# SimonZeng7108/efficientsam3

Hardware: NVIDIA H100
Metric: encoder images/sec @1024^2 (EV-M student forward) (higher is better)
Workload: dtype bf16

## Files before the change

efficientsam3_b200/csrc/gemm_tc.cu:

```cuda
#include <cstdio>
#include <cstdlib>

#include "ptx.cuh"

namespace es3 {

struct GemmArgs {
  int M, N;
  int num_kb;
  int kb_per_tap;
  int tiles_n;
  int conv;
  int H, W, TW, TH, tiles_w, tiles_h;
  int Ctap;
  const float* scale;
  const float* bias;
  int act;
  const bf16* residual;
  long long ldr;
  void* out;
  long long ldo;
  int out_f32;
  int res_f32;
  const float2* rope;
  int rope_cols, rope_H, rope_W, rope_win;
  int ct_cout, ct_H, ct_W;
  int act_after_res;
  int dbg;
};

constexpr int BM = 128;
constexpr int BK = 64;

constexpr int EPI_WARPS = 4;
constexpr int EPI_WARP0 = 4;
constexpr int TMA_WARP = EPI_WARP0 + EPI_WARPS;
constexpr int GEMM_THREADS = (TMA_WARP + 1) * 32;
template <int BN, int STAGES, int CPR>
struct GemmSmem {
  static constexpr int A_BYTES = BM * BK * 2;
  static constexpr int B_BYTES = BN * BK * 2;
  static constexpr int STAGE_BYTES = A_BYTES + B_BYTES;
  static constexpr int ACC_LD = BN + 8;
  static constexpr int OFF_ACC = STAGES * STAGE_BYTES;
  static constexpr int OFF_EPI = OFF_ACC + BM * ACC_LD * 4;
  static constexpr int EPI_TILE_BYTES = 32 * 16 * CPR;
  static constexpr int TOTAL = OFF_EPI + EPI_WARPS * EPI_TILE_BYTES;
};

template <int CPR>
__device__ __forceinline__ uint8_t* epi_chunk(uint8_t* tile, int r, int c) {
  if constexpr (CPR == 4) return tile + r * 64 + ((c ^ ((r >> 1) & 3)) << 4);
  else return tile + r * 32 + ((c ^ ((r >> 2) & 1)) << 4);
}

template <int CPR>
__device__ __forceinline__ void epi_store_rows(uint8_t* tile, const uint4* mine, uint8_t* gbase, long long my_off_bytes,
                                               bool my_valid, int lane) {
  constexpr int RPI = 32 / CPR;
#pragma unroll
  for (int p = 0; p < 4 / CPR; ++p) {
#pragma unroll
    for (int j = 0; j < CPR; ++j) *reinterpret_cast<uint4*>(epi_chunk<CPR>(tile, lane, j)) = mine[p * CPR + j];
    __syncwarp();
#pragma unroll
    for (int j = 0; j < CPR; ++j) {
      const int r = j * RPI + lane / CPR, c = lane % CPR;
      const long long off = __shfl_sync(0xffffffffu, my_off_bytes, r);
      const int ok = __shfl_sync(0xffffffffu, (int)my_valid, r);
      const uint4 u = *reinterpret_cast<const uint4*>(epi_chunk<CPR>(tile, r, c));
      if (ok) *reinterpret_cast<uint4*>(gbase + off + (p * CPR + c) * 16) = u;
    }
    __syncwarp();
  }
}

template <int CPR>
__device__ __forceinline__ void epi_load_rows(uint8_t* tile, uint4* mine, const uint8_t* gbase, long long my_off_bytes,
                                              bool my_valid, int lane) {
  constexpr int RPI = 32 / CPR;
#pragma unroll
  for (int p = 0; p < 4 / CPR; ++p) {
#pragma unroll
    for (int j = 0; j < CPR; ++j) {
      const int r = j * RPI + lane / CPR, c = lane % CPR;
      const long long off = __shfl_sync(0xffffffffu, my_off_bytes, r);
      const int ok = __shfl_sync(0xffffffffu, (int)my_valid, r);
      uint4 u = make_uint4(0u, 0u, 0u, 0u);
      if (ok) u = __ldg(reinterpret_cast<const uint4*>(gbase + off + (p * CPR + c) * 16));
      *reinterpret_cast<uint4*>(epi_chunk<CPR>(tile, r, c)) = u;
    }
    __syncwarp();
#pragma unroll
    for (int j = 0; j < CPR; ++j) mine[p * CPR + j] = *reinterpret_cast<const uint4*>(epi_chunk<CPR>(tile, lane, j));
    __syncwarp();
  }
}

template <int BN, int STAGES, int ACT, int CPR>
__global__ void __launch_bounds__(GEMM_THREADS, 1) gemm_tc_kernel(const __grid_constant__ CUtensorMap tmA,
                                                               const __grid_constant__ CUtensorMap tmB,
                                                               const GemmArgs args, const int num_tiles) {
  static_assert(BN == 32 || BN == 64 || BN == 128, "one warpgroup holds 128 x BN fp32 accumulators in registers");
  extern __shared__ __align__(1024) uint8_t smem[];
  __shared__ __align__(8) uint64_t full_bar[STAGES];
  __shared__ __align__(8) uint64_t empty_bar[STAGES];
  __shared__ __align__(8) uint64_t acc_full_bar;
  __shared__ __align__(8) uint64_t acc_empty_bar;

  using L = GemmSmem<BN, STAGES, CPR>;
  float* acc_s = reinterpret_cast<float*>(smem + L::OFF_ACC);

  const int warp = threadIdx.x >> 5;
  const int lane = threadIdx.x & 31;

  if (threadIdx.x == 0) {
    if (ptx::smem_u32(smem) & 1023u) { printf("es3: gemm_tc dynamic smem base not 1024-byte aligned\n"); __trap(); }
    ptx::prefetch_tmap(&tmA);
    ptx::prefetch_tmap(&tmB);
#pragma unroll
    for (int s = 0; s < STAGES; ++s) {
      ptx::mbar_init(&full_bar[s], 1);
      ptx::mbar_init(&empty_bar[s], 4);
    }
    ptx::mbar_init(&acc_full_bar, 4);
    ptx::mbar_init(&acc_empty_bar, EPI_WARPS);
    ptx::fence_mbar_init();
  }
  __syncthreads();
  const int per_img = args.tiles_w * args.tiles_h;

  if (warp == TMA_WARP) {
    if (lane == 0) {
      int stage = 0;
      uint32_t phase = 0;
      for (int tile = blockIdx.x; tile < num_tiles; tile += gridDim.x) {
        const int n0 = (args.dbg & 8) ? 0 : (tile % args.tiles_n) * BN;
        const int m_tile = (args.dbg & 8) ? 0 : tile / args.tiles_n;
        int img = 0, h0 = 0, w0 = 0;
        if (args.conv) {
          img = m_tile / per_img;
          const int t = m_tile % per_img;
          h0 = (t / args.tiles_w) * args.TH;
          w0 = (t % args.tiles_w) * args.TW;
        }
        for (int kb = 0; kb < args.num_kb; ++kb) {
          ptx::mbar_wait(&empty_bar[stage], phase ^ 1);
          uint8_t* sa = smem + stage * L::STAGE_BYTES;
          uint8_t* sb = sa + L::A_BYTES;
          ptx::mbar_arrive_expect_tx(&full_bar[stage], L::STAGE_BYTES);
          if (args.conv) {
            const int tap = kb / args.kb_per_tap;
            const int kc = kb - tap * args.kb_per_tap;
            const int dy = tap / 3 - 1, dx = tap % 3 - 1;
            ptx::tma_load_4d(&tmA, &full_bar[stage], sa, kc * BK, w0 + dx, h0 + dy, img);
            ptx::tma_load_2d(&tmB, &full_bar[stage], sb, tap * args.Ctap + kc * BK, n0);
          } else {
            ptx::tma_load_2d(&tmA, &full_bar[stage], sa, kb * BK, m_tile * BM);
            ptx::tma_load_2d(&tmB, &full_bar[stage], sb, kb * BK, n0);
          }
          if (++stage == STAGES) { stage = 0; phase ^= 1; }
        }
      }
    }
  } else if (warp < EPI_WARP0) {
    float d[2][BN / 2];
    int stage = 0;
    uint32_t phase = 0;
    uint32_t acc_phase = 0;
    for (int tile = blockIdx.x; tile < num_tiles; tile += gridDim.x) {
      int prev = -1;
      for (int kb = 0; kb < args.num_kb; ++kb) {
        ptx::mbar_wait(&full_bar[stage], phase);
        const uint32_t sa = ptx::smem_u32(smem + stage * L::STAGE_BYTES);
        const uint32_t sb = sa + L::A_BYTES;
        ptx::wg_fence();
#pragma unroll
        for (int k = 0; k < BK / 16; ++k) {
          const uint64_t db = ptx::make_desc_sw128(sb + k * 32);
#pragma unroll
          for (int h = 0; h < 2; ++h) {
            const uint64_t da = ptx::make_desc_sw128(sa + h * 8192 + k * 32);
            if constexpr (BN == 128) ptx::wgmma_m64n128<0, 0>(d[h], da, db, (kb | k) != 0);
            else if constexpr (BN == 64) ptx::wgmma_m64n64<0, 0>(d[h], da, db, (kb | k) != 0);
            else ptx::wgmma_m64n32<0, 0>(d[h], da, db, (kb | k) != 0);
          }
        }
        ptx::wg_commit();
        ptx::wg_wait<1>();
        if (prev >= 0 && lane == 0) ptx::mbar_arrive(&empty_bar[prev]);
        prev = stage;
        if (++stage == STAGES) { stage = 0; phase ^= 1; }
      }
      ptx::wg_wait<0>();
      ptx::wg_fence_regs<BN>(&d[0][0]);
      if (prev >= 0 && lane == 0) ptx::mbar_arrive(&empty_bar[prev]);
      ptx::mbar_wait(&acc_empty_bar, acc_phase ^ 1);
#pragma unroll
      for (int h = 0; h < 2; ++h)
#pragma unroll
        for (int i = 0; i < BN / 2; i += 2) {
          const int row = h * 64 + ptx::wg_frag_row(warp, lane, i), col = ptx::wg_frag_col(lane, i);
          *reinterpret_cast<float2*>(acc_s + row * L::ACC_LD + col) = make_float2(d[h][i], d[h][i + 1]);
        }
      __syncwarp();
      if (lane == 0) ptx::mbar_arrive(&acc_full_bar);
      acc_phase ^= 1;
    }
  } else {
    const int q = warp - EPI_WARP0;
    const int r = q * 32 + lane;
    uint8_t* epi_tile = smem + L::OFF_EPI + q * L::EPI_TILE_BYTES;
    uint32_t acc_phase = 0;
    for (int tile = blockIdx.x; tile < num_tiles; tile += gridDim.x) {
      const int n0 = (tile % args.tiles_n) * BN;
      const int m_tile = tile / args.tiles_n;
      bool valid;
      long long row_off;
      const bool dbg_nostore = (args.dbg & 1) != 0;
      if (args.conv) {
        const int img = m_tile / per_img;
        const int t = m_tile % per_img;
        const int h0 = (t / args.tiles_w) * args.TH, w0 = (t % args.tiles_w) * args.TW;
        const int dy = r / args.TW, dx = r - dy * args.TW;
        const int h = h0 + dy, w = w0 + dx;
        valid = (h < args.H) && (w < args.W);
        row_off = ((long long)img * args.H + h) * args.W + w;
      } else {
        const long long m = (long long)m_tile * BM + r;
        valid = m < args.M;
        row_off = m;
      }

      if (dbg_nostore) valid = false;
      ptx::mbar_wait(&acc_full_bar, acc_phase);

#pragma unroll 1
      for (int c = 0; c < BN / 32; ++c) {
        if (args.dbg & 4) break;
        uint32_t v[32];
        if (args.dbg & 2) {
#pragma unroll
          for (int j = 0; j < 32; ++j) v[j] = __float_as_uint((float)(r + j));
        } else {
          const uint4* src = reinterpret_cast<const uint4*>(acc_s + r * L::ACC_LD + c * 32);
#pragma unroll
          for (int j = 0; j < 8; ++j) {
            const uint4 u = src[j];
            v[4 * j] = u.x; v[4 * j + 1] = u.y; v[4 * j + 2] = u.z; v[4 * j + 3] = u.w;
          }
        }
        const int nb = n0 + c * 32;
        if (valid && nb < args.N && nb + 32 > args.N) {
          const int ncols = args.N - nb;
          const long long out_off = row_off * args.ldo + nb, res_off = row_off * args.ldr + nb;
#pragma unroll
          for (int j = 0; j < 32; ++j) {
            if (j < ncols) {
              float x = __uint_as_float(v[j]);
              if (args.scale != nullptr) x *= __ldg(args.scale + nb + j);
              if (args.bias != nullptr) x += __ldg(args.bias + nb + j);
              if (!args.act_after_res) x = es3_act_t<ACT>(x);
              if (args.residual != nullptr)
                x += args.res_f32 ? __ldg(reinterpret_cast<const float*>(args.residual) + res_off + j)
                                  : __bfloat162float(args.residual[res_off + j]);
              if (args.act_after_res) x = es3_act_t<ACT>(x);
              if (args.out_f32) reinterpret_cast<float*>(args.out)[out_off + j] = x;
              else reinterpret_cast<bf16*>(args.out)[out_off + j] = __float2bfloat16(x);
            }
          }
        } else if (nb + 32 <= args.N) {
          float f[32];
          if (args.scale != nullptr) {
            const float4* sc4 = reinterpret_cast<const float4*>(args.scale + nb);
#pragma unroll
            for (int j = 0; j < 8; ++j) {
              const float4 sc = __ldg(sc4 + j);
              f[4 * j + 0] = __uint_as_float(v[4 * j + 0]) * sc.x;
              f[4 * j + 1] = __uint_as_float(v[4 * j + 1]) * sc.y;
              f[4 * j + 2] = __uint_as_float(v[4 * j + 2]) * sc.z;
              f[4 * j + 3] = __uint_as_float(v[4 * j + 3]) * sc.w;
            }
          } else {
#pragma unroll
            for (int j = 0; j < 32; ++j) f[j] = __uint_as_float(v[j]);
          }
          if (args.bias != nullptr) {
            const float4* bi4 = reinterpret_cast<const float4*>(args.bias + nb);
#pragma unroll
            for (int j = 0; j < 8; ++j) {
              const float4 bi = __ldg(bi4 + j);
              f[4 * j + 0] += bi.x; f[4 * j + 1] += bi.y; f[4 * j + 2] += bi.z; f[4 * j + 3] += bi.w;
            }
          }
          long long out_off = row_off * args.ldo + nb, res_off = row_off * args.ldr + nb;
          if (args.ct_cout) {
            const int pos = nb / args.ct_cout, co = nb - pos * args.ct_cout;
            const long long hw = (long long)args.ct_H * args.ct_W;
            const long long bi = row_off / hw;
            const int rem = (int)(row_off - bi * hw);
            const int hh = rem / args.ct_W, ww = rem - hh * args.ct_W;
            const long long orow = (bi * 2 * args.ct_H + 2 * hh + (pos >> 1)) * (2LL * args.ct_W) + 2 * ww + (pos & 1);
            out_off = orow * args.ldo + co;
            res_off = orow * args.ldr + co;
          }
          if (!args.act_after_res) {
#pragma unroll
            for (int j = 0; j < 32; ++j) f[j] = es3_act_t<ACT>(f[j]);
          }
          if (args.rope != nullptr && nb < args.rope_cols) {
            const int t = (int)(row_off % ((long long)args.rope_H * args.rope_W));
            const int h = t / args.rope_W, w = t - h * args.rope_W;
            const int pidx = args.rope_win ? (h % args.rope_win) * args.rope_win + (w % args.rope_win) : t;
            const float4* tp = reinterpret_cast<const float4*>(args.rope + (long long)pidx * 32 + ((nb & 63) >> 1));
#pragma unroll
            for (int j = 0; j < 8; ++j) {
              const float4 cs = __ldg(tp + j);
              const float x0 = f[4 * j], x1 = f[4 * j + 1], x2 = f[4 * j + 2], x3 = f[4 * j + 3];
              f[4 * j] = x0 * cs.x - x1 * cs.y;
              f[4 * j + 1] = x0 * cs.y + x1 * cs.x;
              f[4 * j + 2] = x2 * cs.z - x3 * cs.w;
              f[4 * j + 3] = x2 * cs.w + x3 * cs.z;
            }
          }
          if (args.residual != nullptr && args.res_f32) {
            const uint8_t* rbase = reinterpret_cast<const uint8_t*>(args.residual);
#pragma unroll
            for (int hf = 0; hf < 2; ++hf) {
              uint4 rr[4];
              epi_load_rows<CPR>(epi_tile, rr, rbase, res_off * 4 + hf * 64, valid, lane);
#pragma unroll
              for (int j = 0; j < 4; ++j) {
                f[hf * 16 + 4 * j + 0] += __uint_as_float(rr[j].x); f[hf * 16 + 4 * j + 1] += __uint_as_float(rr[j].y);
                f[hf * 16 + 4 * j + 2] += __uint_as_float(rr[j].z); f[hf * 16 + 4 * j + 3] += __uint_as_float(rr[j].w);
              }
            }
          } else if (args.residual != nullptr) {
            uint4 rr[4];
            epi_load_rows<CPR>(epi_tile, rr, reinterpret_cast<const uint8_t*>(args.residual), res_off * 2, valid, lane);
#pragma unroll
            for (int j = 0; j < 4; ++j) {
              float rf[8];
              unpack8(rr[j], rf);
#pragma unroll
              for (int e = 0; e < 8; ++e) f[j * 8 + e] += rf[e];
            }
          }
          if (args.act_after_res) {
#pragma unroll
            for (int j = 0; j < 32; ++j) f[j] = es3_act_t<ACT>(f[j]);
          }
          if (args.out_f32) {
            uint8_t* obase = reinterpret_cast<uint8_t*>(args.out);
#pragma unroll
            for (int hf = 0; hf < 2; ++hf) {
              uint4 oo[4];
#pragma unroll
              for (int j = 0; j < 4; ++j)
                oo[j] = make_uint4(__float_as_uint(f[hf * 16 + 4 * j]), __float_as_uint(f[hf * 16 + 4 * j + 1]),
                                   __float_as_uint(f[hf * 16 + 4 * j + 2]), __float_as_uint(f[hf * 16 + 4 * j + 3]));
              epi_store_rows<CPR>(epi_tile, oo, obase, out_off * 4 + hf * 64, valid, lane);
            }
          } else {
            uint4 oo[4];
#pragma unroll
            for (int j = 0; j < 4; ++j) oo[j] = pack8(f + 8 * j);
            epi_store_rows<CPR>(epi_tile, oo, reinterpret_cast<uint8_t*>(args.out), out_off * 2, valid, lane);
          }
        }
      }
      __syncwarp();
      if (lane == 0) ptx::mbar_arrive(&acc_empty_bar);
      acc_phase ^= 1;
    }
  }
}

typedef CUresult (*EncodeTiledFn)(CUtensorMap*, CUtensorMapDataType, cuuint32_t, void*, const cuuint64_t*,
                                  const cuuint64_t*, const cuuint32_t*, const cuuint32_t*, CUtensorMapInterleave,
                                  CUtensorMapSwizzle, CUtensorMapL2promotion, CUtensorMapFloatOOBfill);

static EncodeTiledFn get_encode_fn() {
  static EncodeTiledFn fn = nullptr;
  if (fn) return fn;
  void* p = nullptr;
  cudaDriverEntryPointQueryResult qres;
  cudaError_t e = cudaGetDriverEntryPoint("cuTensorMapEncodeTiled", &p, cudaEnableDefault, &qres);
  if (e != cudaSuccess || qres != cudaDriverEntryPointSuccess || p == nullptr) {
    set_error("cuTensorMapEncodeTiled entry point unavailable (%s)", cudaGetErrorString(e));
    return nullptr;
  }
  fn = reinterpret_cast<EncodeTiledFn>(p);
  return fn;
}

int encode_map(CUtensorMap* map, const void* base, int rank, const uint64_t* dims, const uint64_t* strides_b,
                      const uint32_t* box) {
  EncodeTiledFn fn = get_encode_fn();
  if (!fn) return 1;
  cuuint64_t gdim[5], gstr[5];
  cuuint32_t bx[5], es[5];
  for (int i = 0; i < rank; ++i) { gdim[i] = dims[i]; bx[i] = box[i]; es[i] = 1; }
  for (int i = 0; i < rank - 1; ++i) gstr[i] = strides_b[i];
  CUresult r = fn(map, CU_TENSOR_MAP_DATA_TYPE_BFLOAT16, (cuuint32_t)rank, const_cast<void*>(base), gdim, gstr, bx, es,
                  CU_TENSOR_MAP_INTERLEAVE_NONE, CU_TENSOR_MAP_SWIZZLE_128B, CU_TENSOR_MAP_L2_PROMOTION_L2_256B,
                  CU_TENSOR_MAP_FLOAT_OOB_FILL_NONE);
  if (r != CUDA_SUCCESS) {
    set_error("cuTensorMapEncodeTiled failed (CUresult %d) rank=%d dims=[%llu,%llu,..] box=[%u,%u,..]", (int)r, rank,
              (unsigned long long)dims[0], (unsigned long long)(rank > 1 ? dims[1] : 0), box[0], rank > 1 ? box[1] : 0);
    return 1;
  }
  return 0;
}

template <int BN, int STAGES, int ACT, int CPR>
static int launch_act(const CUtensorMap& tmA, const CUtensorMap& tmB, const GemmArgs& args, int tiles_m,
                      cudaStream_t stream) {
  using L = GemmSmem<BN, STAGES, CPR>;
  static int resident = 0;
  static int sm_count = 0;
  if (resident == 0) {
    ES3_CHECK_CUDA(cudaFuncSetAttribute(gemm_tc_kernel<BN, STAGES, ACT, CPR>, cudaFuncAttributeMaxDynamicSharedMemorySize,
                                        L::TOTAL));
    ES3_CHECK_CUDA(cudaFuncSetAttribute(gemm_tc_kernel<BN, STAGES, ACT, CPR>, cudaFuncAttributePreferredSharedMemoryCarveout,
                                        cudaSharedmemCarveoutMaxShared));
    int dev = 0, occ = 0;
    ES3_CHECK_CUDA(cudaGetDevice(&dev));
    ES3_CHECK_CUDA(cudaDeviceGetAttribute(&sm_count, cudaDevAttrMultiProcessorCount, dev));
    ES3_CHECK_CUDA(cudaOccupancyMaxActiveBlocksPerMultiprocessor(&occ, gemm_tc_kernel<BN, STAGES, ACT, CPR>, GEMM_THREADS, L::TOTAL));
    ES3_REQUIRE(occ >= 1, "gemm_tc_kernel<%d,%d>: does not fit an SM (%d B of dynamic shared memory)", BN, STAGES, L::TOTAL);
    resident = occ < 2 ? 1 : 2;
    if (getenv("ES3_DEBUG_OCCUPANCY"))
      fprintf(stderr, "es3: gemm_tc_kernel<BN=%d,STAGES=%d,ACT=%d,CPR=%d> %d B smem -> %d CTA/SM (runtime occupancy %d)\n", BN, STAGES, ACT,
              CPR, L::TOTAL, resident, occ);
  }
  const int num_tiles = tiles_m * args.tiles_n;
  const int ctas = sm_count * resident;
  dim3 grid((unsigned)(num_tiles < ctas ? num_tiles : ctas));
  gemm_tc_kernel<BN, STAGES, ACT, CPR><<<grid, GEMM_THREADS, L::TOTAL, stream>>>(tmA, tmB, args, num_tiles);
  ES3_LAUNCH_CHECK("gemm_tc_kernel");
  return 0;
}

template <int BN, int STAGES, int CPR>
static int launch(const CUtensorMap& tmA, const CUtensorMap& tmB, const GemmArgs& args, int tiles_m,
                  cudaStream_t stream) {
  switch (args.act) {
    case ACT_NONE: return launch_act<BN, STAGES, ACT_NONE, CPR>(tmA, tmB, args, tiles_m, stream);
    case ACT_RELU: return launch_act<BN, STAGES, ACT_RELU, CPR>(tmA, tmB, args, tiles_m, stream);
    case ACT_HSWISH: return launch_act<BN, STAGES, ACT_HSWISH, CPR>(tmA, tmB, args, tiles_m, stream);
    case ACT_GELU: return launch_act<BN, STAGES, ACT_GELU, CPR>(tmA, tmB, args, tiles_m, stream);
    default: set_error("gemm_tc: activation code %d not instantiated (0,1,2,3)", args.act); return 1;
  }
}

static int pick_bn(int N, int bn_hint, int K = 1 << 30, int act = ACT_NONE) {
  if (bn_hint == 32 || bn_hint == 64 || bn_hint == 128) return bn_hint;
  if (bn_hint == 256) return 128;
  if (K < 512 && N >= 64) {
    if (act == ACT_GELU) return 64;
    return N >= 384 ? 128 : 64;
  }
  if (N % 128 == 0 || N > 1024) return 128;
  if (N % 64 == 0) return 64;
// ... 27 lines not shown
}

extern "C" int es3_gemm_bf16_ex(const void* A, long long lda, const void* W, long long ldw, void* out, long long ldo,
                                int out_f32, int M, int N, int K, const float* scale, const float* bias, int act,
                                const void* residual, long long ldr, int res_f32, const float* rope, int rope_cols,
                                int rope_H, int rope_W, int rope_win, int act_after_res, int bn_hint, void* stream) {
  ES3_REQUIRE(M > 0 && N > 0 && K > 0, "es3_gemm_bf16: bad shape M=%d N=%d K=%d", M, N, K);
  ES3_REQUIRE(rope == nullptr || (rope_cols % 64 == 0 && rope_cols <= N && rope_H > 0 && rope_W > 0 &&
                                  M % (rope_H * rope_W) == 0 && ((uintptr_t)rope & 15) == 0),
              "es3_gemm_bf16_ex: bad rope arguments");
  ES3_REQUIRE(N % 8 == 0, "es3_gemm_bf16: N=%d must be a multiple of 8", N);
  ES3_REQUIRE(N % 32 == 0 || rope == nullptr, "es3_gemm_bf16_ex: the rope epilogue needs N %% 32 == 0 (N=%d)", N);
  ES3_REQUIRE(K % 8 == 0 && lda % 8 == 0 && ldw % 8 == 0, "es3_gemm_bf16: K/lda/ldw must be multiples of 8 (16-byte TMA strides)");
  ES3_REQUIRE(ldo % 8 == 0 && (residual == nullptr || ldr % 8 == 0), "es3_gemm_bf16: ldo/ldr must be multiples of 8");
  ES3_REQUIRE(rope == nullptr || act == ACT_NONE, "es3_gemm_bf16_ex: rope epilogue expects act = none");
  ES3_REQUIRE(((uintptr_t)A & 15) == 0 && ((uintptr_t)W & 15) == 0 && ((uintptr_t)out & 15) == 0,
              "es3_gemm_bf16: pointers must be 16-byte aligned");
  const int bn = (rope != nullptr && bn_hint == 0 && N >= 128) ? 128 : pick_bn(N, bn_hint, K, act);
  CUtensorMap tmA, tmB;
  {
    uint64_t dims[2] = {(uint64_t)K, (uint64_t)M};
    uint64_t str[1] = {(uint64_t)lda * 2};
    uint32_t box[2] = {(uint32_t)BK, (uint32_t)BM};
    if (encode_map(&tmA, A, 2, dims, str, box)) return 1;
  }
  {
    uint64_t dims[2] = {(uint64_t)K, (uint64_t)N};
    uint64_t str[1] = {(uint64_t)ldw * 2};
    uint32_t box[2] = {(uint32_t)BK, (uint32_t)bn};
    if (encode_map(&tmB, W, 2, dims, str, box)) return 1;
  }
  GemmArgs a;
  memset(&a, 0, sizeof(a));
  { const char* e = getenv("ES3_GEMM_DBG"); if (e) a.dbg = atoi(e); }
  a.M = M; a.N = N;
  a.num_kb = ceil_div(K, BK);
  a.kb_per_tap = a.num_kb;
  a.tiles_n = ceil_div(N, bn);
  a.conv = 0;
  a.scale = scale; a.bias = bias; a.act = act;
  a.residual = (const bf16*)residual; a.ldr = ldr; a.res_f32 = res_f32;
  a.rope = (const float2*)rope; a.rope_cols = rope_cols; a.rope_H = rope_H; a.rope_W = rope_W; a.rope_win = rope_win;
  a.act_after_res = act_after_res;
  a.out = out; a.ldo = ldo; a.out_f32 = out_f32;
  return dispatch(bn, tmA, tmB, a, ceil_div(M, BM), (cudaStream_t)stream);
}

extern "C" int es3_conv3x3_bf16(const void* x, const void* W, void* out, int out_f32, int B, int H, int Wd, int C,
                                int N, const float* scale, const float* bias, int act, const void* residual,
                                int bn_hint, void* stream) {
  ES3_REQUIRE(B > 0 && H > 0 && Wd > 0, "es3_conv3x3_bf16: bad shape");
  ES3_REQUIRE(C % 8 == 0 && N % 32 == 0, "es3_conv3x3_bf16: need C %% 8 == 0 and N %% 32 == 0 (C=%d N=%d)", C, N);
  const int bn = pick_bn(N, bn_hint);
  int TW = 8;
  if (Wd % 32 == 0) TW = 32; else if (Wd % 16 == 0) TW = 16;
  const int TH = BM / TW;
  CUtensorMap tmA, tmB;
  {
    uint64_t dims[4] = {(uint64_t)C, (uint64_t)Wd, (uint64_t)H, (uint64_t)B};
    uint64_t str[3] = {(uint64_t)C * 2, (uint64_t)Wd * C * 2, (uint64_t)H * Wd * C * 2};
    uint32_t box[4] = {(uint32_t)BK, (uint32_t)TW, (uint32_t)TH, 1u};
    if (encode_map(&tmA, x, 4, dims, str, box)) return 1;
  }
  {
    uint64_t dims[2] = {(uint64_t)9 * C, (uint64_t)N};
    uint64_t str[1] = {(uint64_t)9 * C * 2};
    uint32_t box[2] = {(uint32_t)BK, (uint32_t)bn};
    if (encode_map(&tmB, W, 2, dims, str, box)) return 1;
  }
  GemmArgs a;
  memset(&a, 0, sizeof(a));
  { const char* e = getenv("ES3_GEMM_DBG"); if (e) a.dbg = atoi(e); }
  a.M = B * H * Wd; a.N = N;
  a.kb_per_tap = ceil_div(C, BK);
  a.num_kb = 9 * a.kb_per_tap;
  a.tiles_n = ceil_div(N, bn);
  a.conv = 1;
  a.H = H; a.W = Wd; a.TW = TW; a.TH = TH;
  a.tiles_w = ceil_div(Wd, TW); a.tiles_h = ceil_div(H, TH);
  a.Ctap = C;
  a.scale = scale; a.bias = bias; a.act = act;
  a.residual = (const bf16*)residual; a.ldr = N;
  a.out = out; a.ldo = N; a.out_f32 = out_f32;
  return dispatch(bn, tmA, tmB, a, B * a.tiles_w * a.tiles_h, (cudaStream_t)stream);
}

extern "C" int es3_convt2x2_bf16(const void* x, const void* Wt, void* out, int out_f32, int B, int H, int Wd, int Cin,
                                 int Cout, const float* bias4, int act, const void* residual, int res_f32,
                                 int act_after_res, void* stream) {
  ES3_REQUIRE(Cout % 32 == 0 && Cin % 8 == 0, "es3_convt2x2_bf16: need Cout %% 32 == 0 and Cin %% 8 == 0 (Cin=%d Cout=%d)", Cin, Cout);
  const int M = B * H * Wd, N = 4 * Cout, K = Cin;
  const int bn = pick_bn(N, 0);
  CUtensorMap tmA, tmB;
  {
    uint64_t dims[2] = {(uint64_t)K, (uint64_t)M};
    uint64_t str[1] = {(uint64_t)K * 2};
    uint32_t box[2] = {(uint32_t)BK, (uint32_t)BM};
    if (encode_map(&tmA, x, 2, dims, str, box)) return 1;
  }
  {
    uint64_t dims[2] = {(uint64_t)K, (uint64_t)N};
    uint64_t str[1] = {(uint64_t)K * 2};
    uint32_t box[2] = {(uint32_t)BK, (uint32_t)bn};
    if (encode_map(&tmB, Wt, 2, dims, str, box)) return 1;
  }
  GemmArgs a;
  memset(&a, 0, sizeof(a));
  { const char* e = getenv("ES3_GEMM_DBG"); if (e) a.dbg = atoi(e); }
  a.M = M; a.N = N;
  a.num_kb = ceil_div(K, BK);
  a.kb_per_tap = a.num_kb;
  a.tiles_n = ceil_div(N, bn);
  a.bias = bias4; a.act = act;
  a.residual = (const bf16*)residual; a.ldr = Cout; a.res_f32 = res_f32;
  a.out = out; a.ldo = Cout; a.out_f32 = out_f32;
  a.ct_cout = Cout; a.ct_H = H; a.ct_W = Wd; a.act_after_res = act_after_res;
  return dispatch(bn, tmA, tmB, a, ceil_div(M, BM), (cudaStream_t)stream);
}
```

efficientsam3_b200/csrc/ptx.cuh:

```cuda
#pragma once
#include "common.cuh"

namespace es3 {
int encode_map(CUtensorMap* map, const void* base, int rank, const uint64_t* dims, const uint64_t* strides_b, const uint32_t* box);
}

namespace ptx {

__device__ __forceinline__ uint32_t smem_u32(const void* p) {
  return static_cast<uint32_t>(__cvta_generic_to_shared(p));
}

__device__ __forceinline__ void ldsm_x4(uint32_t addr, uint32_t& r0, uint32_t& r1, uint32_t& r2, uint32_t& r3) {
  asm volatile("ldmatrix.sync.aligned.m8n8.x4.shared.b16 {%0,%1,%2,%3}, [%4];"
               : "=r"(r0), "=r"(r1), "=r"(r2), "=r"(r3) : "r"(addr));
}
__device__ __forceinline__ void mma_16816(float* d, const uint32_t* a, uint32_t b0, uint32_t b1) {
  asm volatile(
      "mma.sync.aligned.m16n8k16.row.col.f32.bf16.bf16.f32 {%0,%1,%2,%3}, {%4,%5,%6,%7}, {%8,%9}, {%0,%1,%2,%3};"
      : "+f"(d[0]), "+f"(d[1]), "+f"(d[2]), "+f"(d[3])
      : "r"(a[0]), "r"(a[1]), "r"(a[2]), "r"(a[3]), "r"(b0), "r"(b1));
}
__device__ __forceinline__ void mma_1688(float* d, uint32_t a0, uint32_t a1, uint32_t b0) {
  asm volatile(
// ... 6 lines not shown
  asm volatile("mbarrier.init.shared::cta.b64 [%0], %1;" ::"r"(smem_u32(bar)), "r"(count) : "memory");
}
__device__ __forceinline__ void fence_mbar_init() {
  asm volatile("fence.mbarrier_init.release.cluster;" ::: "memory");
}
__device__ __forceinline__ void fence_proxy_async() {
  asm volatile("fence.proxy.async.shared::cta;" ::: "memory");
}
__device__ __forceinline__ void mbar_arrive_expect_tx(uint64_t* bar, uint32_t bytes) {
  asm volatile("mbarrier.arrive.expect_tx.shared::cta.b64 _, [%0], %1;" ::"r"(smem_u32(bar)), "r"(bytes) : "memory");
}
__device__ __forceinline__ void mbar_arrive(uint64_t* bar) {
  asm volatile("mbarrier.arrive.shared::cta.b64 _, [%0];" ::"r"(smem_u32(bar)) : "memory");
}
__device__ __forceinline__ bool mbar_try_wait(uint64_t* bar, uint32_t parity) {
  uint32_t done;
  asm volatile(
      "{\n\t.reg .pred p;\n\t"
      "mbarrier.try_wait.parity.shared::cta.b64 p, [%1], %2;\n\t"
      "selp.u32 %0, 1, 0, p;\n\t}"
      : "=r"(done)
      : "r"(smem_u32(bar)), "r"(parity)
      : "memory");
  return done != 0;
}
__device__ __forceinline__ void mbar_wait(uint64_t* bar, uint32_t parity) {
  if (mbar_try_wait(bar, parity)) return;
  long long t0 = clock64();
  while (!mbar_try_wait(bar, parity)) {
    if (clock64() - t0 > 4000000000LL) __trap();
  }
}

__device__ __forceinline__ void prefetch_tmap(const void* tmap) {
  asm volatile("prefetch.tensormap [%0];" ::"l"(reinterpret_cast<uint64_t>(tmap)) : "memory");
}
__device__ __forceinline__ void tma_load_2d(const void* tmap, uint64_t* bar, void* smem, int c0, int c1) {
  asm volatile(
      "cp.async.bulk.tensor.2d.shared::cluster.global.mbarrier::complete_tx::bytes [%0], [%1, {%3, %4}], [%2];"
      ::"r"(smem_u32(smem)), "l"(reinterpret_cast<uint64_t>(tmap)), "r"(smem_u32(bar)), "r"(c0), "r"(c1)
      : "memory");
}
__device__ __forceinline__ void tma_load_3d(const void* tmap, uint64_t* bar, void* smem, int c0, int c1, int c2) {
  asm volatile(
      "cp.async.bulk.tensor.3d.shared::cluster.global.mbarrier::complete_tx::bytes [%0], [%1, {%3, %4, %5}], [%2];"
      ::"r"(smem_u32(smem)), "l"(reinterpret_cast<uint64_t>(tmap)), "r"(smem_u32(bar)), "r"(c0), "r"(c1), "r"(c2)
      : "memory");
}
__device__ __forceinline__ void tma_load_4d(const void* tmap, uint64_t* bar, void* smem, int c0, int c1, int c2,
                                            int c3) {
  asm volatile(
      "cp.async.bulk.tensor.4d.shared::cluster.global.mbarrier::complete_tx::bytes [%0], [%1, {%3, %4, %5, %6}], [%2];"
      ::"r"(smem_u32(smem)), "l"(reinterpret_cast<uint64_t>(tmap)), "r"(smem_u32(bar)), "r"(c0), "r"(c1), "r"(c2),
      "r"(c3)
      : "memory");
}

__device__ __forceinline__ int wg_frag_row(int warp_in_group, int lane, int i) {
  return 16 * warp_in_group + (lane >> 2) + 8 * ((i >> 1) & 1);
}
__device__ __forceinline__ int wg_frag_col(int lane, int i) { return 8 * (i >> 2) + 2 * (lane & 3) + (i & 1); }

__device__ __forceinline__ void wg_fence() { asm volatile("wgmma.fence.sync.aligned;" ::: "memory"); }
__device__ __forceinline__ void wg_commit() { asm volatile("wgmma.commit_group.sync.aligned;" ::: "memory"); }
template <int N>
__device__ __forceinline__ void wg_wait() { asm volatile("wgmma.wait_group.sync.aligned %0;" ::"n"(N) : "memory"); }
template <int R>
__device__ __forceinline__ void wg_fence_regs(float* d) {
#pragma unroll
  for (int i = 0; i < R; ++i) asm volatile("" : "+f"(d[i])::"memory");
}

__device__ __forceinline__ void named_bar(int id, int threads) {
  asm volatile("bar.sync %0, %1;" ::"r"(id), "r"(threads) : "memory");
}

template <int N>
__device__ __forceinline__ void setmaxnreg_dec() { asm volatile("setmaxnreg.dec.sync.aligned.u32 %0;" ::"n"(N)); }
template <int N>
__device__ __forceinline__ void setmaxnreg_inc() { asm volatile("setmaxnreg.inc.sync.aligned.u32 %0;" ::"n"(N)); }

__device__ __forceinline__ uint64_t make_desc_sw128(uint32_t smem_addr) {
  uint64_t d = 0;
  d |= (uint64_t)((smem_addr & 0x3FFFFu) >> 4);
  d |= (uint64_t)1 << 16;
  d |= (uint64_t)(1024u >> 4) << 32;
  d |= (uint64_t)1 << 62;
  return d;
}
__device__ __forceinline__ uint64_t desc_advance(uint64_t d, uint32_t off) {
  return ((d >> 32) << 32) | (uint32_t)((uint32_t)d + (off >> 4));
}

template <int TA, int TB>
__device__ __forceinline__ void wgmma_m64n32(float* d, uint64_t desc_a, uint64_t desc_b, uint32_t accumulate) {
  asm volatile(
      "{\n\t.reg .pred p;\n\t"
      "setp.ne.b32 p, %18, 0;\n\t"
      "wgmma.mma_async.sync.aligned.m64n32k16.f32.bf16.bf16 "
      "{%0, %1, %2, %3, %4, %5, %6, %7, %8, %9, %10, %11, %12, %13, %14, %15}, "
      "%16, %17, p, 1, 1, %19, %20;\n\t}"
      : "+f"(d[0]), "+f"(d[1]), "+f"(d[2]), "+f"(d[3]), "+f"(d[4]), "+f"(d[5]), "+f"(d[6]), "+f"(d[7]), "+f"(d[8]), "+f"(d[9]), "+f"(d[10]), "+f"(d[11]), "+f"(d[12]), "+f"(d[13]), "+f"(d[14]), "+f"(d[15])
      : "l"(desc_a), "l"(desc_b), "r"(accumulate), "n"(TA), "n"(TB)
      : "memory");
}

template <int TA, int TB>
__device__ __forceinline__ void wgmma_m64n64(float* d, uint64_t desc_a, uint64_t desc_b, uint32_t accumulate) {
// ... 88 lines not shown
```

Before: 4055.

## Restructure GEMM into ping-pong consumer warpgroups with fused in-register epilogue

Replaces the separate MMA warpgroup plus epilogue warps, which handed off through a full fp32 accumulator tile in shared memory, with two consumer warpgroups that alternate tiles (ping-pong via named barriers). Each consumer runs its own epilogue from registers through a small per-warp staging buffer, and register allocation is rebalanced with setmaxnreg between one producer warpgroup and the consumers. It also prefetches residual lines into L2 before the mainloop and drops the debug flag paths. The intent is to overlap one warpgroup's epilogue with the other's MMA and cut the accumulator shared-memory round trip. In exchange, residency is forced to one CTA per SM and the register pressure on the consumers rises.

Measured after the change: 4180 (median of 6 runs). 1.03x the previous value.

```diff
diff --git a/efficientsam3_b200/csrc/gemm_tc.cu b/efficientsam3_b200/csrc/gemm_tc.cu
--- a/efficientsam3_b200/csrc/gemm_tc.cu
+++ b/efficientsam3_b200/csrc/gemm_tc.cu
@@ -26,26 +26,25 @@
   int rope_cols, rope_H, rope_W, rope_win;
   int ct_cout, ct_H, ct_W;
   int act_after_res;
-  int dbg;
 };
 
 constexpr int BM = 128;
 constexpr int BK = 64;
 
-constexpr int EPI_WARPS = 4;
-constexpr int EPI_WARP0 = 4;
-constexpr int TMA_WARP = EPI_WARP0 + EPI_WARPS;
-constexpr int GEMM_THREADS = (TMA_WARP + 1) * 32;
+constexpr int GEMM_THREADS = 3 * 128;
+constexpr int CONSUMER_WARP0 = 4;
+constexpr int PRODUCER_REGS = 40, CONSUMER_REGS = 232;
+constexpr int FRAG_LD = 40;
 template <int BN, int STAGES, int CPR>
 struct GemmSmem {
   static constexpr int A_BYTES = BM * BK * 2;
   static constexpr int B_BYTES = BN * BK * 2;
   static constexpr int STAGE_BYTES = A_BYTES + B_BYTES;
-  static constexpr int ACC_LD = BN + 8;
-  static constexpr int OFF_ACC = STAGES * STAGE_BYTES;
-  static constexpr int OFF_EPI = OFF_ACC + BM * ACC_LD * 4;
+  static constexpr int FRAG_BYTES = 32 * FRAG_LD * 4;
   static constexpr int EPI_TILE_BYTES = 32 * 16 * CPR;
-  static constexpr int TOTAL = OFF_EPI + EPI_WARPS * EPI_TILE_BYTES;
+  static constexpr int WARP_BYTES = FRAG_BYTES + EPI_TILE_BYTES;
+  static constexpr int OFF_EPI = STAGES * STAGE_BYTES;
+  static constexpr int TOTAL = OFF_EPI + 8 * WARP_BYTES;
 };
 
 template <int CPR>
@@ -94,6 +93,128 @@
 #pragma unroll
     for (int j = 0; j < CPR; ++j) mine[p * CPR + j] = *reinterpret_cast<const uint4*>(epi_chunk<CPR>(tile, lane, j));
     __syncwarp();
+  }
+}
+
+template <int ACT, int CPR>
+__device__ __forceinline__ void epi_row_chunk(const GemmArgs& args, const uint32_t* v, int nb, long long row_off, bool valid,
+                                              uint8_t* epi_tile, int lane) {
+  if (valid && nb < args.N && nb + 32 > args.N) {
+    const int ncols = args.N - nb;
+    const long long out_off = row_off * args.ldo + nb, res_off = row_off * args.ldr + nb;
+#pragma unroll
+    for (int j = 0; j < 32; ++j) {
+      if (j < ncols) {
+        float x = __uint_as_float(v[j]);
+        if (args.scale != nullptr) x *= __ldg(args.scale + nb + j);
+        if (args.bias != nullptr) x += __ldg(args.bias + nb + j);
+        if (!args.act_after_res) x = es3_act_t<ACT>(x);
+        if (args.residual != nullptr)
+          x += args.res_f32 ? __ldg(reinterpret_cast<const float*>(args.residual) + res_off + j)
+                            : __bfloat162float(args.residual[res_off + j]);
+        if (args.act_after_res) x = es3_act_t<ACT>(x);
+        if (args.out_f32) reinterpret_cast<float*>(args.out)[out_off + j] = x;
+        else reinterpret_cast<bf16*>(args.out)[out_off + j] = __float2bfloat16(x);
+      }
+    }
+  } else if (nb + 32 <= args.N) {
+    float f[32];
+    if (args.scale != nullptr) {
+      const float4* sc4 = reinterpret_cast<const float4*>(args.scale + nb);
+#pragma unroll
+      for (int j = 0; j < 8; ++j) {
+        const float4 sc = __ldg(sc4 + j);
+        f[4 * j + 0] = __uint_as_float(v[4 * j + 0]) * sc.x;
+        f[4 * j + 1] = __uint_as_float(v[4 * j + 1]) * sc.y;
+        f[4 * j + 2] = __uint_as_float(v[4 * j + 2]) * sc.z;
+        f[4 * j + 3] = __uint_as_float(v[4 * j + 3]) * sc.w;
+      }
+    } else {
+#pragma unroll
+      for (int j = 0; j < 32; ++j) f[j] = __uint_as_float(v[j]);
+    }
+    if (args.bias != nullptr) {
+      const float4* bi4 = reinterpret_cast<const float4*>(args.bias + nb);
+#pragma unroll
+      for (int j = 0; j < 8; ++j) {
+        const float4 bi = __ldg(bi4 + j);
+        f[4 * j + 0] += bi.x; f[4 * j + 1] += bi.y; f[4 * j + 2] += bi.z; f[4 * j + 3] += bi.w;
+      }
+    }
+    long long out_off = row_off * args.ldo + nb, res_off = row_off * args.ldr + nb;
+    if (args.ct_cout) {
+      const int pos = nb / args.ct_cout, co = nb - pos * args.ct_cout;
+      const long long hw = (long long)args.ct_H * args.ct_W;
+      const long long bi = row_off / hw;
+      const int rem = (int)(row_off - bi * hw);
+      const int hh = rem / args.ct_W, ww = rem - hh * args.ct_W;
+      const long long orow = (bi * 2 * args.ct_H + 2 * hh + (pos >> 1)) * (2LL * args.ct_W) + 2 * ww + (pos & 1);
+      out_off = orow * args.ldo + co;
+      res_off = orow * args.ldr + co;
+    }
+    if (!args.act_after_res) {
+#pragma unroll
+      for (int j = 0; j < 32; ++j) f[j] = es3_act_t<ACT>(f[j]);
+    }
+    if (args.rope != nullptr && nb < args.rope_cols) {
+      const int t = (int)(row_off % ((long long)args.rope_H * args.rope_W));
+      const int h = t / args.rope_W, w = t - h * args.rope_W;
+      const int pidx = args.rope_win ? (h % args.rope_win) * args.rope_win + (w % args.rope_win) : t;
+      const float4* tp = reinterpret_cast<const float4*>(args.rope + (long long)pidx * 32 + ((nb & 63) >> 1));
+#pragma unroll
+      for (int j = 0; j < 8; ++j) {
+        const float4 cs = __ldg(tp + j);
+        const float x0 = f[4 * j], x1 = f[4 * j + 1], x2 = f[4 * j + 2], x3 = f[4 * j + 3];
+        f[4 * j] = x0 * cs.x - x1 * cs.y;
+        f[4 * j + 1] = x0 * cs.y + x1 * cs.x;
+        f[4 * j + 2] = x2 * cs.z - x3 * cs.w;
+        f[4 * j + 3] = x2 * cs.w + x3 * cs.z;
+      }
+    }
+    if (args.residual != nullptr && args.res_f32) {
+      const uint8_t* rbase = reinterpret_cast<const uint8_t*>(args.residual);
+#pragma unroll
+      for (int hf = 0; hf < 2; ++hf) {
+        uint4 rr[4];
+        epi_load_rows<CPR>(epi_tile, rr, rbase, res_off * 4 + hf * 64, valid, lane);
+#pragma unroll
+        for (int j = 0; j < 4; ++j) {
+          f[hf * 16 + 4 * j + 0] += __uint_as_float(rr[j].x); f[hf * 16 + 4 * j + 1] += __uint_as_float(rr[j].y);
+          f[hf * 16 + 4 * j + 2] += __uint_as_float(rr[j].z); f[hf * 16 + 4 * j + 3] += __uint_as_float(rr[j].w);
+        }
+      }
+    } else if (args.residual != nullptr) {
+      uint4 rr[4];
+      epi_load_rows<CPR>(epi_tile, rr, reinterpret_cast<const uint8_t*>(args.residual), res_off * 2, valid, lane);
+#pragma unroll
+      for (int j = 0; j < 4; ++j) {
+        float rf[8];
+        unpack8(rr[j], rf);
+#pragma unroll
+        for (int e = 0; e < 8; ++e) f[j * 8 + e] += rf[e];
+      }
+    }
+    if (args.act_after_res) {
+#pragma unroll
+      for (int j = 0; j < 32; ++j) f[j] = es3_act_t<ACT>(f[j]);
+    }
+    if (args.out_f32) {
+      uint8_t* obase = reinterpret_cast<uint8_t*>(args.out);
+#pragma unroll
+      for (int hf = 0; hf < 2; ++hf) {
+        uint4 oo[4];
+#pragma unroll
+        for (int j = 0; j < 4; ++j)
+          oo[j] = make_uint4(__float_as_uint(f[hf * 16 + 4 * j]), __float_as_uint(f[hf * 16 + 4 * j + 1]),
+                             __float_as_uint(f[hf * 16 + 4 * j + 2]), __float_as_uint(f[hf * 16 + 4 * j + 3]));
+        epi_store_rows<CPR>(epi_tile, oo, obase, out_off * 4 + hf * 64, valid, lane);
+      }
+    } else {
+      uint4 oo[4];
+#pragma unroll
+      for (int j = 0; j < 4; ++j) oo[j] = pack8(f + 8 * j);
+      epi_store_rows<CPR>(epi_tile, oo, reinterpret_cast<uint8_t*>(args.out), out_off * 2, valid, lane);
+    }
   }
 }
 
@@ -105,11 +226,8 @@
   extern __shared__ __align__(1024) uint8_t smem[];
   __shared__ __align__(8) uint64_t full_bar[STAGES];
   __shared__ __align__(8) uint64_t empty_bar[STAGES];
-  __shared__ __align__(8) uint64_t acc_full_bar;
-  __shared__ __align__(8) uint64_t acc_empty_bar;
 
   using L = GemmSmem<BN, STAGES, CPR>;
-  float* acc_s = reinterpret_cast<float*>(smem + L::OFF_ACC);
 
   const int warp = threadIdx.x >> 5;
   const int lane = threadIdx.x & 31;
@@ -123,20 +241,19 @@
       ptx::mbar_init(&full_bar[s], 1);
       ptx::mbar_init(&empty_bar[s], 4);
     }
-    ptx::mbar_init(&acc_full_bar, 4);
-    ptx::mbar_init(&acc_empty_bar, EPI_WARPS);
     ptx::fence_mbar_init();
   }
   __syncthreads();
   const int per_img = args.tiles_w * args.tiles_h;
 
-  if (warp == TMA_WARP) {
-    if (lane == 0) {
+  if (warp < CONSUMER_WARP0) {
+    ptx::setmaxnreg_dec<PRODUCER_REGS>();
+    if (warp == 0 && lane == 0) {
       int stage = 0;
       uint32_t phase = 0;
       for (int tile = blockIdx.x; tile < num_tiles; tile += gridDim.x) {
-        const int n0 = (args.dbg & 8) ? 0 : (tile % args.tiles_n) * BN;
-        const int m_tile = (args.dbg & 8) ? 0 : tile / args.tiles_n;
+        const int n0 = (tile % args.tiles_n) * BN;
+        const int m_tile = tile / args.tiles_n;
         int img = 0, h0 = 0, w0 = 0;
         if (args.conv) {
           img = m_tile / per_img;
@@ -163,215 +280,98 @@
         }
       }
     }
-  } else if (warp < EPI_WARP0) {
-    float d[2][BN / 2];
-    int stage = 0;
-    uint32_t phase = 0;
-    uint32_t acc_phase = 0;
-    for (int tile = blockIdx.x; tile < num_tiles; tile += gridDim.x) {
-      int prev = -1;
-      for (int kb = 0; kb < args.num_kb; ++kb) {
-        ptx::mbar_wait(&full_bar[stage], phase);
-        const uint32_t sa = ptx::smem_u32(smem + stage * L::STAGE_BYTES);
-        const uint32_t sb = sa + L::A_BYTES;
-        ptx::wg_fence();
-#pragma unroll
-        for (int k = 0; k < BK / 16; ++k) {
-          const uint64_t db = ptx::make_desc_sw128(sb + k * 32);
-#pragma unroll
-          for (int h = 0; h < 2; ++h) {
-            const uint64_t da = ptx::make_desc_sw128(sa + h * 8192 + k * 32);
-            if constexpr (BN == 128) ptx::wgmma_m64n128<0, 0>(d[h], da, db, (kb | k) != 0);
-            else if constexpr (BN == 64) ptx::wgmma_m64n64<0, 0>(d[h], da, db, (kb | k) != 0);
-            else ptx::wgmma_m64n32<0, 0>(d[h], da, db, (kb | k) != 0);
+    return;
+  }
+
+  ptx::setmaxnreg_inc<CONSUMER_REGS>();
+  const int cons = (warp >> 2) - 1;
+  const int q = warp & 3;
+  const int my_tiles = (int)blockIdx.x < num_tiles ? (num_tiles - 1 - (int)blockIdx.x) / (int)gridDim.x + 1 : 0;
+  uint8_t* wbase = smem + L::OFF_EPI + (warp - CONSUMER_WARP0) * L::WARP_BYTES;
+  float* frag = reinterpret_cast<float*>(wbase);
+  uint8_t* epi_tile = wbase + L::FRAG_BYTES;
+  const int r = (lane >> 4) * 64 + 16 * q + (lane & 15);
+  float d[2][BN / 2];
+
+  for (int i = cons; i < my_tiles; i += 2) {
+    const int tile = (int)blockIdx.x + i * (int)gridDim.x;
+    const int n0 = (tile % args.tiles_n) * BN;
+    const int m_tile = tile / args.tiles_n;
+    bool valid;
+    long long row_off;
+    if (args.conv) {
+      const int img = m_tile / per_img;
+      const int t = m_tile % per_img;
+      const int h0 = (t / args.tiles_w) * args.TH, w0 = (t % args.tiles_w) * args.TW;
+      const int dy = r / args.TW, dx = r - dy * args.TW;
+      const int h = h0 + dy, w = w0 + dx;
+      valid = (h < args.H) && (w < args.W);
+      row_off = ((long long)img * args.H + h) * args.W + w;
+    } else {
+      const long long m = (long long)m_tile * BM + r;
+      valid = m < args.M;
+      row_off = m;
+    }
+    if (args.residual != nullptr && !args.ct_cout && valid) {
+      const int esz = args.res_f32 ? 4 : 2;
+      const int ncols = args.N - n0 < BN ? args.N - n0 : BN;
+      const uintptr_t first = reinterpret_cast<uintptr_t>(args.residual) + (uintptr_t)((row_off * args.ldr + n0) * esz);
+      const uintptr_t last = first + (uintptr_t)(ncols * esz - 1);
+      for (uintptr_t line = first & ~(uintptr_t)127; line <= last; line += 128) ptx::prefetch_l2(reinterpret_cast<const void*>(line));
+    }
+    if (i > 0) ptx::named_bar(1 + cons, 2 * 128);
+    uint32_t it = (uint32_t)i * (uint32_t)args.num_kb;
+    int prev = -1;
+    for (int kb = 0; kb < args.num_kb; ++kb, ++it) {
+      const int stage = (int)(it % STAGES);
+      ptx::mbar_wait(&full_bar[stage], (it / STAGES) & 1);
+      const uint32_t sa = ptx::smem_u32(smem + stage * L::STAGE_BYTES);
+      const uint32_t sb = sa + L::A_BYTES;
+      ptx::wg_fence();
+#pragma unroll
+      for (int k = 0; k < BK / 16; ++k) {
+        const uint64_t db = ptx::make_desc_sw128(sb + k * 32);
+#pragma unroll
+        for (int h = 0; h < 2; ++h) {
+          const uint64_t da = ptx::make_desc_sw128(sa + h * 8192 + k * 32);
+          if constexpr (BN == 128) ptx::wgmma_m64n128<0, 0>(d[h], da, db, (kb | k) != 0);
+          else if constexpr (BN == 64) ptx::wgmma_m64n64<0, 0>(d[h], da, db, (kb | k) != 0);
+          else ptx::wgmma_m64n32<0, 0>(d[h], da, db, (kb | k) != 0);
+        }
+      }
+      ptx::wg_commit();
+      ptx::wg_wait<1>();
+      if (prev >= 0 && lane == 0) ptx::mbar_arrive(&empty_bar[prev]);
+      prev = stage;
+    }
+    if (i + 1 < my_tiles) ptx::named_bar_arrive(2 - cons, 2 * 128);
+    ptx::wg_wait<0>();
+    ptx::wg_fence_regs<BN>(&d[0][0]);
+    if (prev >= 0 && lane == 0) ptx::mbar_arrive(&empty_bar[prev]);
+
+#pragma unroll 1
+    for (int c = 0; c < BN / 32; ++c) {
+#pragma unroll
+      for (int cc = 0; cc < BN / 32; ++cc) {
+        if (cc != c) continue;
+#pragma unroll
+        for (int h = 0; h < 2; ++h)
+#pragma unroll
+          for (int i = 16 * cc; i < 16 * cc + 16; i += 2) {
+            const int lr = 16 * h + ptx::wg_frag_row(0, lane, i), col = ptx::wg_frag_col(lane, i) - 32 * cc;
+            *reinterpret_cast<float2*>(frag + lr * FRAG_LD + col) = make_float2(d[h][i], d[h][i + 1]);
           }
-        }
-        ptx::wg_commit();
-        ptx::wg_wait<1>();
-        if (prev >= 0 && lane == 0) ptx::mbar_arrive(&empty_bar[prev]);
-        prev = stage;
-        if (++stage == STAGES) { stage = 0; phase ^= 1; }
-      }
-      ptx::wg_wait<0>();
-      ptx::wg_fence_regs<BN>(&d[0][0]);
-      if (prev >= 0 && lane == 0) ptx::mbar_arrive(&empty_bar[prev]);
-      ptx::mbar_wait(&acc_empty_bar, acc_phase ^ 1);
-#pragma unroll
-      for (int h = 0; h < 2; ++h)
-#pragma unroll
-        for (int i = 0; i < BN / 2; i += 2) {
-          const int row = h * 64 + ptx::wg_frag_row(warp, lane, i), col = ptx::wg_frag_col(lane, i);
-          *reinterpret_cast<float2*>(acc_s + row * L::ACC_LD + col) = make_float2(d[h][i], d[h][i + 1]);
-        }
+      }
       __syncwarp();
-      if (lane == 0) ptx::mbar_arrive(&acc_full_bar);
-      acc_phase ^= 1;
-    }
-  } else {
-    const int q = warp - EPI_WARP0;
-    const int r = q * 32 + lane;
-    uint8_t* epi_tile = smem + L::OFF_EPI + q * L::EPI_TILE_BYTES;
-    uint32_t acc_phase = 0;
-    for (int tile = blockIdx.x; tile < num_tiles; tile += gridDim.x) {
-      const int n0 = (tile % args.tiles_n) * BN;
-      const int m_tile = tile / args.tiles_n;
-      bool valid;
-      long long row_off;
-      const bool dbg_nostore = (args.dbg & 1) != 0;
-      if (args.conv) {
-        const int img = m_tile / per_img;
-        const int t = m_tile % per_img;
-        const int h0 = (t / args.tiles_w) * args.TH, w0 = (t % args.tiles_w) * args.TW;
-        const int dy = r / args.TW, dx = r - dy * args.TW;
-        const int h = h0 + dy, w = w0 + dx;
-        valid = (h < args.H) && (w < args.W);
-        row_off = ((long long)img * args.H + h) * args.W + w;
-      } else {
-        const long long m = (long long)m_tile * BM + r;
-        valid = m < args.M;
-        row_off = m;
-      }
-
-      if (dbg_nostore) valid = false;
-      ptx::mbar_wait(&acc_full_bar, acc_phase);
-
-#pragma unroll 1
-      for (int c = 0; c < BN / 32; ++c) {
-        if (args.dbg & 4) break;
-        uint32_t v[32];
-        if (args.dbg & 2) {
-#pragma unroll
-          for (int j = 0; j < 32; ++j) v[j] = __float_as_uint((float)(r + j));
-        } else {
-          const uint4* src = reinterpret_cast<const uint4*>(acc_s + r * L::ACC_LD + c * 32);
-#pragma unroll
-          for (int j = 0; j < 8; ++j) {
-            const uint4 u = src[j];
-            v[4 * j] = u.x; v[4 * j + 1] = u.y; v[4 * j + 2] = u.z; v[4 * j + 3] = u.w;
-          }
-        }
-        const int nb = n0 + c * 32;
-        if (valid && nb < args.N && nb + 32 > args.N) {
-          const int ncols = args.N - nb;
-          const long long out_off = row_off * args.ldo + nb, res_off = row_off * args.ldr + nb;
-#pragma unroll
-          for (int j = 0; j < 32; ++j) {
-            if (j < ncols) {
-              float x = __uint_as_float(v[j]);
-              if (args.scale != nullptr) x *= __ldg(args.scale + nb + j);
-              if (args.bias != nullptr) x += __ldg(args.bias + nb + j);
-              if (!args.act_after_res) x = es3_act_t<ACT>(x);
-              if (args.residual != nullptr)
-                x += args.res_f32 ? __ldg(reinterpret_cast<const float*>(args.residual) + res_off + j)
-                                  : __bfloat162float(args.residual[res_off + j]);
-              if (args.act_after_res) x = es3_act_t<ACT>(x);
-              if (args.out_f32) reinterpret_cast<float*>(args.out)[out_off + j] = x;
-              else reinterpret_cast<bf16*>(args.out)[out_off + j] = __float2bfloat16(x);
-            }
-          }
-        } else if (nb + 32 <= args.N) {
-          float f[32];
-          if (args.scale != nullptr) {
-            const float4* sc4 = reinterpret_cast<const float4*>(args.scale + nb);
-#pragma unroll
-            for (int j = 0; j < 8; ++j) {
-              const float4 sc = __ldg(sc4 + j);
-              f[4 * j + 0] = __uint_as_float(v[4 * j + 0]) * sc.x;
-              f[4 * j + 1] = __uint_as_float(v[4 * j + 1]) * sc.y;
-              f[4 * j + 2] = __uint_as_float(v[4 * j + 2]) * sc.z;
-              f[4 * j + 3] = __uint_as_float(v[4 * j + 3]) * sc.w;
-            }
-          } else {
-#pragma unroll
-            for (int j = 0; j < 32; ++j) f[j] = __uint_as_float(v[j]);
-          }
-          if (args.bias != nullptr) {
-            const float4* bi4 = reinterpret_cast<const float4*>(args.bias + nb);
-#pragma unroll
-            for (int j = 0; j < 8; ++j) {
-              const float4 bi = __ldg(bi4 + j);
-              f[4 * j + 0] += bi.x; f[4 * j + 1] += bi.y; f[4 * j + 2] += bi.z; f[4 * j + 3] += bi.w;
-            }
-          }
-          long long out_off = row_off * args.ldo + nb, res_off = row_off * args.ldr + nb;
-          if (args.ct_cout) {
-            const int pos = nb / args.ct_cout, co = nb - pos * args.ct_cout;
-            const long long hw = (long long)args.ct_H * args.ct_W;
-            const long long bi = row_off / hw;
-            const int rem = (int)(row_off - bi * hw);
-            const int hh = rem / args.ct_W, ww = rem - hh * args.ct_W;
-            const long long orow = (bi * 2 * args.ct_H + 2 * hh + (pos >> 1)) * (2LL * args.ct_W) + 2 * ww + (pos & 1);
-            out_off = orow * args.ldo + co;
-            res_off = orow * args.ldr + co;
-          }
-          if (!args.act_after_res) {
-#pragma unroll
-            for (int j = 0; j < 32; ++j) f[j] = es3_act_t<ACT>(f[j]);
-          }
-          if (args.rope != nullptr && nb < args.rope_cols) {
-            const int t = (int)(row_off % ((long long)args.rope_H * args.rope_W));
-            const int h = t / args.rope_W, w = t - h * args.rope_W;
-            const int pidx = args.rope_win ? (h % args.rope_win) * args.rope_win + (w % args.rope_win) : t;
-            const float4* tp = reinterpret_cast<const float4*>(args.rope + (long long)pidx * 32 + ((nb & 63) >> 1));
-#pragma unroll
-            for (int j = 0; j < 8; ++j) {
-              const float4 cs = __ldg(tp + j);
-              const float x0 = f[4 * j], x1 = f[4 * j + 1], x2 = f[4 * j + 2], x3 = f[4 * j + 3];
-              f[4 * j] = x0 * cs.x - x1 * cs.y;
-              f[4 * j + 1] = x0 * cs.y + x1 * cs.x;
-              f[4 * j + 2] = x2 * cs.z - x3 * cs.w;
-              f[4 * j + 3] = x2 * cs.w + x3 * cs.z;
-            }
-          }
-          if (args.residual != nullptr && args.res_f32) {
-            const uint8_t* rbase = reinterpret_cast<const uint8_t*>(args.residual);
-#pragma unroll
-            for (int hf = 0; hf < 2; ++hf) {
-              uint4 rr[4];
-              epi_load_rows<CPR>(epi_tile, rr, rbase, res_off * 4 + hf * 64, valid, lane);
-#pragma unroll
-              for (int j = 0; j < 4; ++j) {
-                f[hf * 16 + 4 * j + 0] += __uint_as_float(rr[j].x); f[hf * 16 + 4 * j + 1] += __uint_as_float(rr[j].y);
-                f[hf * 16 + 4 * j + 2] += __uint_as_float(rr[j].z); f[hf * 16 + 4 * j + 3] += __uint_as_float(rr[j].w);
-              }
-            }
-          } else if (args.residual != nullptr) {
-            uint4 rr[4];
-            epi_load_rows<CPR>(epi_tile, rr, reinterpret_cast<const uint8_t*>(args.residual), res_off * 2, valid, lane);
-#pragma unroll
-            for (int j = 0; j < 4; ++j) {
-              float rf[8];
-              unpack8(rr[j], rf);
-#pragma unroll
-              for (int e = 0; e < 8; ++e) f[j * 8 + e] += rf[e];
-            }
-          }
-          if (args.act_after_res) {
-#pragma unroll
-            for (int j = 0; j < 32; ++j) f[j] = es3_act_t<ACT>(f[j]);
-          }
-          if (args.out_f32) {
-            uint8_t* obase = reinterpret_cast<uint8_t*>(args.out);
-#pragma unroll
-            for (int hf = 0; hf < 2; ++hf) {
-              uint4 oo[4];
-#pragma unroll
-              for (int j = 0; j < 4; ++j)
-                oo[j] = make_uint4(__float_as_uint(f[hf * 16 + 4 * j]), __float_as_uint(f[hf * 16 + 4 * j + 1]),
-                                   __float_as_uint(f[hf * 16 + 4 * j + 2]), __float_as_uint(f[hf * 16 + 4 * j + 3]));
-              epi_store_rows<CPR>(epi_tile, oo, obase, out_off * 4 + hf * 64, valid, lane);
-            }
-          } else {
-            uint4 oo[4];
-#pragma unroll
-            for (int j = 0; j < 4; ++j) oo[j] = pack8(f + 8 * j);
-            epi_store_rows<CPR>(epi_tile, oo, reinterpret_cast<uint8_t*>(args.out), out_off * 2, valid, lane);
-          }
-        }
+      uint32_t v[32];
+      const uint4* src = reinterpret_cast<const uint4*>(frag + lane * FRAG_LD);
+#pragma unroll
+      for (int j = 0; j < 8; ++j) {
+        const uint4 u = src[j];
+        v[4 * j] = u.x; v[4 * j + 1] = u.y; v[4 * j + 2] = u.z; v[4 * j + 3] = u.w;
       }
       __syncwarp();
-      if (lane == 0) ptx::mbar_arrive(&acc_empty_bar);
-      acc_phase ^= 1;
+      epi_row_chunk<ACT, CPR>(args, v, n0 + c * 32, row_off, valid, epi_tile, lane);
     }
   }
 }
@@ -429,7 +429,7 @@
     ES3_CHECK_CUDA(cudaDeviceGetAttribute(&sm_count, cudaDevAttrMultiProcessorCount, dev));
     ES3_CHECK_CUDA(cudaOccupancyMaxActiveBlocksPerMultiprocessor(&occ, gemm_tc_kernel<BN, STAGES, ACT, CPR>, GEMM_THREADS, L::TOTAL));
     ES3_REQUIRE(occ >= 1, "gemm_tc_kernel<%d,%d>: does not fit an SM (%d B of dynamic shared memory)", BN, STAGES, L::TOTAL);
-    resident = occ < 2 ? 1 : 2;
+    resident = 1;
     if (getenv("ES3_DEBUG_OCCUPANCY"))
       fprintf(stderr, "es3: gemm_tc_kernel<BN=%d,STAGES=%d,ACT=%d,CPR=%d> %d B smem -> %d CTA/SM (runtime occupancy %d)\n", BN, STAGES, ACT,
               CPR, L::TOTAL, resident, occ);
@@ -523,7 +523,6 @@
   }
   GemmArgs a;
   memset(&a, 0, sizeof(a));
-  { const char* e = getenv("ES3_GEMM_DBG"); if (e) a.dbg = atoi(e); }
   a.M = M; a.N = N;
   a.num_kb = ceil_div(K, BK);
   a.kb_per_tap = a.num_kb;
@@ -561,7 +560,6 @@
   }
   GemmArgs a;
   memset(&a, 0, sizeof(a));
-  { const char* e = getenv("ES3_GEMM_DBG"); if (e) a.dbg = atoi(e); }
   a.M = B * H * Wd; a.N = N;
   a.kb_per_tap = ceil_div(C, BK);
   a.num_kb = 9 * a.kb_per_tap;
@@ -597,7 +595,6 @@
   }
   GemmArgs a;
   memset(&a, 0, sizeof(a));
-  { const char* e = getenv("ES3_GEMM_DBG"); if (e) a.dbg = atoi(e); }
   a.M = M; a.N = N;
   a.num_kb = ceil_div(K, BK);
   a.kb_per_tap = a.num_kb;
diff --git a/efficientsam3_b200/csrc/ptx.cuh b/efficientsam3_b200/csrc/ptx.cuh
--- a/efficientsam3_b200/csrc/ptx.cuh
+++ b/efficientsam3_b200/csrc/ptx.cuh
@@ -62,6 +62,9 @@
   }
 }
 
+__device__ __forceinline__ void prefetch_l2(const void* p) {
+  asm volatile("prefetch.global.L2 [%0];" ::"l"(p));
+}
 __device__ __forceinline__ void prefetch_tmap(const void* tmap) {
   asm volatile("prefetch.tensormap [%0];" ::"l"(reinterpret_cast<uint64_t>(tmap)) : "memory");
 }
@@ -104,6 +107,9 @@
 __device__ __forceinline__ void named_bar(int id, int threads) {
   asm volatile("bar.sync %0, %1;" ::"r"(id), "r"(threads) : "memory");
 }
+__device__ __forceinline__ void named_bar_arrive(int id, int threads) {
+  asm volatile("bar.arrive %0, %1;" ::"r"(id), "r"(threads) : "memory");
+}
 
 template <int N>
 __device__ __forceinline__ void setmaxnreg_dec() { asm volatile("setmaxnreg.dec.sync.aligned.u32 %0;" ::"n"(N)); }
```
